# leggedrobotics/art_planner

Measured on AMD Instinct MI355X. Metric: validated states/sec on 400x400@0.04m map (sample + validity check), higher is better.
Workload: dtype f32; 1 GPU; C2: lazy_prm_star_min_update front end, 400x400@0.04m Perlin terrain (seed 1234) + 12 obstacles, YAML robot, batch sampler + validity checker; map=400x400@0.04, lanes=1

## Files before the change

### art_planner_amd/_capi.py

```python
from __future__ import annotations

import ctypes as C
import os

_HERE = os.path.dirname(os.path.abspath(__file__))
LIB_PATH = os.path.join(_HERE, "csrc", "libartp.so")
if os.environ.get("ARTP_LIB"):
    LIB_PATH = os.path.abspath(os.environ["ARTP_LIB"])

SYMBOLS = [
    "artp_params_defaults", "artp_params_yaml", "artp_status_string", "artp_last_error",
    "artp_device_arch", "artp_create", "artp_destroy", "artp_set_stream", "artp_use_own_stream",
    "artp_synchronize", "artp_set_lane", "artp_get_lane", "artp_map_version",
    "artp_upload_layer", "artp_update_layer_rect", "artp_update_layer_rects", "artp_check_boxes", "artp_check_boxes_dev",
    "artp_validate_states", "artp_validate_states_dev", "artp_set_persistent_latency", "artp_persistent_latency_stats", "artp_upload_sampler_layers",
    "artp_sample_states", "artp_sample_states_dev", "artp_sample_and_validate_dev",
    "artp_sample_and_validate", "artp_reachability_map", "artp_reachability_map_dev", "artp_reachability_poses",
    "artp_reachability_halo", "artp_field_params_defaults", "artp_field_compute", "artp_field_dist", "artp_field_dist_dev",
    "artp_field_path", "artp_field_edge_costs", "artp_field_stats", "artp_field_update", "artp_field_update_stats",
    "artp_field_destroy", "artp_field_learned_params_defaults", "artp_field_compute_learned", "artp_field_learned_stats",
    "artp_field_update_learned", "artp_field_learned_update_stats", "artp_field_block_moves", "artp_field_unblock",
    "artp_field_blocked_count", "artp_field_blocked", "artp_field_plan", "artp_field_plan_stats", "artp_field_plan_round_tile_runs",
    "artp_clearance_params_defaults", "artp_clearance_map", "artp_clearance_map_dev",
    "artp_field_clearance_params_defaults", "artp_field_compute_clearance", "artp_field_clearance",
    "artp_field_update_clearance", "artp_field_clearance_update_stats",
    "artp_check_motions_last_valid", "artp_check_motions_last_valid_dev",
    "artp_set_z_bounds", "artp_set_few_edges", "artp_set_edge_passes", "artp_cost_set_fc_path", "artp_check_motions", "artp_check_motions_dev", "artp_check_edges_interp",
    "artp_check_edges_interp_dev", "artp_compact_valid_dev", "artp_compact_valid_indices_dev", "artp_sample_states_at_dev",
    "artp_pack_edge_results_dev", "artp_cost_update_map_dev", "artp_pack_valid_bits_dev", "artp_indices_from_bits_dev",
    "artp_materialise_from_bits_dev",
    "artp_shard_first_index", "artp_group_create", "artp_group_unique_id", "artp_group_create_rank",
    "artp_group_destroy", "artp_group_last_error", "artp_group_world_size", "artp_group_local_count",
    "artp_group_rank", "artp_group_ctx", "artp_group_ranks_seen", "artp_group_configure",
    "artp_group_sample_and_validate_step", "artp_group_step_buffers", "artp_group_exchange_edges",
    "artp_group_edge_buffers", "artp_group_synchronize", "artp_group_abort",
    "artp_algorithmic_vertices_dev",
    "artp_debug_pipeline_counters", "artp_debug_partner_table", "artp_roadmap_params_defaults",
    "artp_roadmap_build", "artp_roadmap_stats", "artp_roadmap_export", "artp_roadmap_solve", "artp_roadmap_destroy",
    "artp_roadmap_revalidate", "artp_roadmap_set_query", "artp_roadmap_simplify_path", "artp_roadmap_grow",
    "artp_roadmap_solve_until", "artp_roadmap_set_density_map", "artp_roadmap_solve_many",
    "artp_preprocessed_reweight_dev",
    "artp_preprocess_params_defaults", "artp_preprocess_params_yaml", "artp_preprocess_map",
    "artp_preprocess_map_ex", "artp_preprocessed_change",
    "artp_preprocessed_get_layer", "artp_preprocessed_install", "artp_preprocessed_destroy",
    "artp_inpaint_layer", "artp_cost_set_hole_filling", "artp_cost_set_external_query",
    "artp_cost_blob_bytes", "artp_cost_load_weights", "artp_cost_update_map_layer",
    "artp_cost_update_map", "artp_cost_query", "artp_cost_query_dev", "artp_cost_get_features", "artp_cost_debug_query_cells",
    "artp_cost_debug_forms",
    "artp_cost_blob_bytes_version", "artp_cost_feature_channels", "artp_cost_get_features_c", "artp_cost_fc_path", "artp_set_r3_extent", "artp_telea_inpaint_u8",
    "artp_tree_params_defaults", "artp_tree_create", "artp_tree_grow", "artp_tree_solve", "artp_tree_stats",
# ... 192 lines not shown
    L.artp_field_destroy.restype = None
    L.artp_field_block_moves.argtypes = [vp, vp, vp, sz, C.POINTER(C.c_uint64)]
    L.artp_field_unblock.argtypes = [vp, vp, C.POINTER(C.c_uint64)]
    L.artp_field_blocked_count.argtypes = [vp, C.POINTER(C.c_uint64)]
    L.artp_field_blocked.argtypes = [vp, vp]
    L.artp_field_plan.argtypes = [vp, vp, sz, i32, vp, vp, vp, vp, vp, sz]
    L.artp_field_plan_stats.argtypes = [vp, C.POINTER(FieldPlanStats)]
    L.artp_field_plan_round_tile_runs.argtypes = [vp, vp, sz, C.POINTER(sz)]
    L.artp_clearance_params_defaults.argtypes = [C.POINTER(ClearanceParams)]
    L.artp_clearance_params_defaults.restype = None
    for name in ("artp_clearance_map", "artp_clearance_map_dev"):
        getattr(L, name).argtypes = [vp, C.POINTER(ClearanceParams), i32, i32, i32, vp, i32, vp]
    L.artp_field_clearance_params_defaults.argtypes = [C.POINTER(FieldClearanceParams)]
    L.artp_field_clearance_params_defaults.restype = None
    L.artp_field_compute_clearance.argtypes = [vp, C.POINTER(FieldClearanceParams), i32, vp, vp, i32, vp, sz, i32,
                                               C.POINTER(vp)]
    L.artp_field_clearance.argtypes = [vp, vp]
    L.artp_field_update_clearance.argtypes = [vp, vp, i32, vp, i32]
    L.artp_field_clearance_update_stats.argtypes = [vp, C.POINTER(FieldClearanceUpdateStats)]
    L.artp_map_version.argtypes = [vp]
    L.artp_map_version.restype = C.c_uint64
    L.artp_set_z_bounds.argtypes = [vp, dbl, dbl]
    L.artp_set_few_edges.argtypes = [vp, i32]
    L.artp_set_persistent_latency.argtypes = [vp, i32]
    L.artp_persistent_latency_stats.argtypes = [vp, C.POINTER(u64 * 2)]
    L.artp_set_edge_passes.argtypes = [vp, i32, i32]
    L.artp_cost_set_fc_path.argtypes = [vp, i32]
    for name in ("artp_check_motions_last_valid", "artp_check_motions_last_valid_dev"):
        getattr(L, name).argtypes = [vp, vp, vp, sz, vp, vp, vp]
    for name in ("artp_check_motions", "artp_check_motions_dev"):
        getattr(L, name).argtypes = [vp, vp, vp, sz, vp]
    for name in ("artp_check_edges_interp", "artp_check_edges_interp_dev"):
        getattr(L, name).argtypes = [vp, vp, vp, sz, vp, vp]
    L.artp_compact_valid_dev.argtypes = [vp, vp, vp, sz, vp, vp]
    L.artp_compact_valid_indices_dev.argtypes = [vp, vp, sz, vp, vp]
    L.artp_sample_states_at_dev.argtypes = [vp, u64, u64, vp, vp, sz, vp]
    L.artp_materialise_from_bits_dev.argtypes = [vp, u64, vp, i32, sz, sz, vp, sz, vp, vp]
    L.artp_pack_edge_results_dev.argtypes = [vp, vp, vp, vp, vp, sz, vp, vp]
    L.artp_pack_valid_bits_dev.argtypes = [vp, vp, sz, vp]
    L.artp_indices_from_bits_dev.argtypes = [vp, vp, sz, vp, vp]
    L.artp_shard_first_index.argtypes = [u64, i32, i32, u64]
    L.artp_shard_first_index.restype = u64
    L.artp_group_create.argtypes = [C.POINTER(i32), i32, C.POINTER(Params), i32, C.POINTER(vp)]
    L.artp_group_unique_id.argtypes = [vp]
    L.artp_group_create_rank.argtypes = [i32, i32, i32, vp, C.POINTER(Params), C.POINTER(vp)]
    L.artp_group_destroy.argtypes = [vp]
# ... 100 lines not shown
```

### art_planner_amd/context.py

```python
from __future__ import annotations

import ctypes as C
from typing import Optional

import numpy as np

from . import _capi


def make_params(kind="yaml", **overrides) -> _capi.Params:
    L = _capi.load()
    p = _capi.Params()
    (L.artp_params_yaml if kind == "yaml" else L.artp_params_defaults)(C.byref(p))
    for k, v in overrides.items():
        setattr(p, k, v)
    return p


def _f32F(a) -> np.ndarray:
    return np.asfortranarray(a, dtype=np.float32)


class Context:

# ... 86 lines not shown
        valid = np.empty(n, np.uint8)
        detail = np.empty((n, 6), np.int8) if want_detail else None
        self._chk(self.L.artp_validate_states(self.h, se3.ctypes.data, n, valid.ctypes.data,
                                              detail.ctypes.data if want_detail else None),
                  "artp_validate_states")
        return (valid, detail) if want_detail else valid

    def sample_states(self, seed, first_index, n):
        out = np.empty((n, 7), np.float64)
        self._chk(self.L.artp_sample_states(self.h, seed, first_index, n, out.ctypes.data),
                  "artp_sample_states")
        return out

    def set_persistent_latency(self, enabled=True):
        self._chk(self.L.artp_set_persistent_latency(self.h, 1 if enabled else 0), "artp_set_persistent_latency")

    def persistent_latency_stats(self):
        out = (C.c_uint64 * 2)()
        self._chk(self.L.artp_persistent_latency_stats(self.h, C.byref(out)), "artp_persistent_latency_stats")
        return {"launches": int(out[0]), "requests": int(out[1])}

    def set_few_edges(self, enabled=True):
        self._chk(self.L.artp_set_few_edges(self.h, 1 if enabled else 0), "artp_set_few_edges")

    def set_edge_passes(self, two_pass=True, coarse_stride=0):
        self._chk(self.L.artp_set_edge_passes(self.h, 1 if two_pass else 0, coarse_stride), "artp_set_edge_passes")

    def check_motions(self, s1, s2):
        s1 = np.ascontiguousarray(s1, np.float64).reshape(-1, 7)
        s2 = np.ascontiguousarray(s2, np.float64).reshape(-1, 7)
        valid = np.empty(s1.shape[0], np.uint8)
        self._chk(self.L.artp_check_motions(self.h, s1.ctypes.data, s2.ctypes.data, s1.shape[0],
                                            valid.ctypes.data), "artp_check_motions")
        return valid

    def set_z_bounds(self, z_low, z_high):
        self._chk(self.L.artp_set_z_bounds(self.h, float(z_low), float(z_high)), "artp_set_z_bounds")
        self.z_bounds = (float(z_low), float(z_high))

    def set_r3_extent(self, max_extent):
        self._chk(self.L.artp_set_r3_extent(self.h, float(max_extent)), "artp_set_r3_extent")

    def check_motions_last_valid(self, s1, s2):
        s1 = np.ascontiguousarray(s1, np.float64).reshape(-1, 7)
        s2 = np.ascontiguousarray(s2, np.float64).reshape(-1, 7)
        n = s1.shape[0]
# ... 169 lines not shown

    def check_boxes_dev(self, slot, box, poses_t, hit_t, ec_t=None):
        box = np.ascontiguousarray(box, np.float32)
        self._chk(self.L.artp_check_boxes_dev(self.h, slot, box.ctypes.data, poses_t.data_ptr(),
                                              poses_t.shape[0], hit_t.data_ptr(),
                                              ec_t.data_ptr() if ec_t is not None else None),
                  "artp_check_boxes_dev")

    def compact_valid_dev(self, se3_t, valid_t, out_t, count_t):
        self._chk(self.L.artp_compact_valid_dev(self.h, se3_t.data_ptr(), valid_t.data_ptr(), se3_t.shape[0],
                                                out_t.data_ptr(), count_t.data_ptr()), "artp_compact_valid_dev")

    def algorithmic_vertices_dev(self, se3_t) -> int:
        v = C.c_uint64(0)
        self._chk(self.L.artp_algorithmic_vertices_dev(self.h, se3_t.data_ptr(), se3_t.shape[0], C.byref(v)),
                  "artp_algorithmic_vertices_dev")
        return v.value

    def pipeline_counters(self):
        out = (C.c_uint64 * 8)()
        self._chk(self.L.artp_debug_pipeline_counters(self.h, C.byref(out)), "artp_debug_pipeline_counters")
        return {"torso_queued": out[0], "feet_queued": out[4], "exact_grouping": out[1], "feet_plane_stage": out[5],
                "feet_partner_pass": out[6],
                "torso_staged_pass": out[2]}

    def partner_table(self, slot, shape):
        r = C.c_int(0)
        self._chk(self.L.artp_debug_partner_table(self.h, slot, None, 0, C.byref(r)), "artp_debug_partner_table")
        if r.value == 0:
            return None, 0
        out = np.empty(shape[0] * shape[1], np.uint8)
        self._chk(self.L.artp_debug_partner_table(self.h, slot, out.ctypes.data, out.size, C.byref(r)),
                  "artp_debug_partner_table")
        return out.reshape(shape[1], shape[0]), r.value

    def preprocess_map(self, elevation, len_x, len_y, pos_x=0.0, pos_y=0.0, traversability=None, kind="yaml",
                       observed=None, vertices=None, **overrides):
        p = _capi.PreprocessParams()
        (self.L.artp_preprocess_params_yaml if kind == "yaml" else self.L.artp_preprocess_params_defaults)(C.byref(p))
        for k, v in overrides.items():
            setattr(p, k, v)
        e = _f32F(elevation)
        t = _f32F(traversability) if traversability is not None else None
        o = _f32F(observed) if observed is not None else None
        vs = np.ascontiguousarray(vertices, np.float64).reshape(-1, 7) if vertices is not None else None
        inp = _capi.PreprocessInputs(e.ctypes.data, t.ctypes.data if t is not None else None,
                                     o.ctypes.data if o is not None else None,
# ... 174 lines not shown
```

### art_planner_amd/csrc/artp_capi.hip

```cpp
#include "../../include/artp_c.h"

#include <hip/hip_runtime.h>
#include <hipcub/hipcub.hpp>

#include <cmath>
#include <cstdio>
#include <atomic>
#include <chrono>
#include <cstdlib>
#include <cstring>
#include <mutex>
#include <string>
#include <array>
#include <vector>

#include "device_scratch.h"
#include "pipeline.h"
#include "cost_kernels.h"

using namespace artp;

#define ARTP_FEW_STATES 16
#define ARTP_SVC_MAX_STATES 2
#define FEW_EDGE_S1 0
#define FEW_EDGE_S2 (ARTP_FEW_EDGES * 7 * sizeof(double))
#define FEW_EDGE_LAST_T (2 * ARTP_FEW_EDGES * 7 * sizeof(double))
#define FEW_EDGE_LAST_STATE (FEW_EDGE_LAST_T + ARTP_FEW_EDGES * sizeof(double))
#define FEW_EDGE_AUX (FEW_EDGE_LAST_STATE + ARTP_FEW_EDGES * 7 * sizeof(double))
#define FEW_EDGE_STATUS (FEW_EDGE_AUX + ARTP_FEW_EDGES * sizeof(uint32_t))
#define FEW_EDGE_BLOCK_BYTES (FEW_EDGE_STATUS + ARTP_FEW_EDGES)
#define ARTP_MAX_LANES 4

struct artp_ctx {
  int device = 0;
  hipStream_t own_stream = nullptr;
  hipStream_t stream = nullptr;
  artp_params params{};
  RobotDev robot{};
  MapGeom geom{};
  bool have_geom = false;
  std::atomic<uint64_t> map_version{0};
  FieldDev field[2]{};
  float* field_data[2] = {nullptr, nullptr};
  size_t field_elems[2] = {0, 0};
  bool have_field[2] = {false, false};
  void* rect_stage_host = nullptr;
  void* rect_stage_dev = nullptr;
  size_t rect_stage_cap = 0;
  hipEvent_t rect_stage_done = nullptr;
  hipEvent_t map_written = nullptr;
  hipEvent_t lane_mark[4] = {nullptr, nullptr, nullptr, nullptr};
  uint64_t map_write_seq = 0;
  uint64_t map_seen[4] = {0, 0, 0, 0};
  SamplerDev sampler{};
// ... 57 lines not shown
  char* pin_edges = nullptr;
  char* pin_edges_dev = nullptr;
  FewEdgeSync* d_few_sync = nullptr;
  int* d_error = nullptr;
  unsigned long long* d_count = nullptr;
  void* tmp[8] = {nullptr, nullptr, nullptr, nullptr, nullptr, nullptr, nullptr, nullptr};
  size_t tmp_cap[8] = {0, 0, 0, 0, 0, 0, 0, 0};
  void* cub_tmp = nullptr;
  size_t cub_cap = 0;
  int32_t* clear_offs[33] = {};
  uint32_t clear_n[33] = {};
  struct lane_state {
    bool init = false;
    hipStream_t own_stream = nullptr, stream = nullptr;
    unsigned long long* d_count = nullptr;
    int* d_error = nullptr;
    void* tmp[8] = {nullptr, nullptr, nullptr, nullptr, nullptr, nullptr, nullptr, nullptr};
    size_t tmp_cap[8] = {0, 0, 0, 0, 0, 0, 0, 0};
    void* cub_tmp = nullptr;
    size_t cub_cap = 0;
  };
  lane_state lanes[ARTP_MAX_LANES];
  int cur_lane = 0;
  bool have_weights = false;
  int cost_net = 0;
  half8* d_convw[5] = {nullptr, nullptr, nullptr, nullptr, nullptr};
  float* d_convb[5] = {nullptr, nullptr, nullptr, nullptr, nullptr};
  float* d_c12 = nullptr;
  unsigned char* d_c12m = nullptr;
  int conv12_mfma = 1;
  half8* d_convw_chunk[3] = {nullptr, nullptr, nullptr};
  half8* d_convw_p32 = nullptr;
  float* d_fc = nullptr;
  char* d_fc_mfma = nullptr;
  int feet_dense = 0;
  double r3_extent_override = 0.0;
  int fc_mfma = 1;
  int fc_selfcheck = -1;
  float fc_selfcheck_err = 0.f;
  half_t* d_act[2] = {nullptr, nullptr};
  size_t act_cap = 0;
  half_t* d_feat = nullptr;
  size_t feat_cap = 0;
  float* d_map_f32 = nullptr;
  size_t map_cap = 0;
  CostMapGeom cost_geom{};
// ... 182 lines not shown
  std::lock_guard<std::mutex> lock(mu);
  int* have = nullptr;
  for (auto& e : set)
    if (e.first.first == c->device && e.first.second == fn) have = &e.second;
  if (have && *have >= (int)bytes) return ARTP_OK;
  HIP_TRY(c, hipFuncSetAttribute(fn, hipFuncAttributeMaxDynamicSharedMemorySize, (int)bytes));
  if (have)
    *have = (int)bytes;
  else
    set.push_back({{c->device, fn}, (int)bytes});
  return ARTP_OK;
}

#define ARTP_OPT_IN(c, kernel, bytes)                                                       \
  do {                                                                                      \
    const int _rc = opt_in_lds((c), reinterpret_cast<const void*>(kernel), (bytes));        \
    if (_rc != ARTP_OK) return _rc;                                                         \
  } while (0)

int set_kernel_lds(artp_ctx* c) {
  ARTP_OPT_IN(c, check_boxes_kernel<1>, lds_full(c));
  ARTP_OPT_IN(c, validate_states_kernel<1>, lds_full(c));
  ARTP_OPT_IN(c, plane_stage_kernel<1>, lds_full(c));
  ARTP_OPT_IN(c, validate_few_kernel, lds_few(c));
  ARTP_OPT_IN(c, check_motions_few_kernel, lds_few(c));
  ARTP_OPT_IN(c, validate_service_kernel, lds_few(c));
  ARTP_OPT_IN(c, check_motions_pool_kernel, lds_few(c));
  ARTP_OPT_IN(c, (resolve_boxes_kernel<ARTP_WAVES_PER_BLOCK, 64, 3>), lds_scan(c));
  ARTP_OPT_IN(c, (resolve_boxes_kernel<ARTP_WAVES_PER_BLOCK, 16, 1>), lds_feet(c));
  ARTP_OPT_IN(c, (resolve_boxes_kernel<ARTP_WAVES_PER_BLOCK, 64, 2>), lds_feet_wave(c));
  return ARTP_OK;
}

int grid_full(const artp_ctx* c, size_t tasks) {
  size_t per_cu = (160 * 1024) / (lds_full(c) ? lds_full(c) : 1);
  if (per_cu > 16) per_cu = 16;
  if (per_cu < 1) per_cu = 1;
  size_t g = (size_t)c->n_cus * per_cu;
  if (tasks && tasks < g) g = tasks;
  return (int)(g ? g : 1);
}
int grid_scan(const artp_ctx* c, size_t lds) {
  size_t per_cu = (160 * 1024) / (lds ? lds : 1);
  if (per_cu > 8) per_cu = 8;
  if (per_cu < 1) per_cu = 1;
  return (int)((size_t)c->n_cus * per_cu);
// ... 157 lines not shown
  t.has_nan = f.has_nan;
  t.has_nonfinite = c->layer_has_nonfinite[slot];
  {
    unsigned off[ARTP_STRIDE_LEVELS + 1] = {0};
    for (int l = 0; l < ARTP_STRIDE_LEVELS; ++l) {
      const int s = 2 << l;
      off[l + 1] = off[l] + (unsigned)(((f.nW + s - 1) / s) * ((f.nD + s - 1) / s));
    }
    t.st = c->stride_buf[slot];
    t.st_off1 = off[1];
    t.st_off2 = off[2];
    hipLaunchKernelGGL(stride_tables_kernel, dim3((off[3] + 255) / 256), dim3(256), 0, c->stream, t.mm, t.fl, t.stride,
                       f.nW, f.nD, off[1], off[2], off[3], c->stride_buf[slot]);
    HIP_TRY(c, hipGetLastError());
  }
  const int rc_partner = pr ? partner_update_end(c, slot, *pr) : build_partner_table_full(c, slot);
  if (rc_partner != ARTP_OK) return rc_partner;
  t.valid = 1;
  return ARTP_OK;
}

int ensure_recs(artp_ctx* c, size_t n) { return ensure_tmp(c, 7, n * sizeof(PoseRec)); }

int launch_validate_pipeline(artp_ctx* c, const double* se3, size_t n, uint8_t* valid, bool recs_ready = false) {
  if (n >= (1ull << 32)) {
    c->last_error = "batch too large (state index is 32 bit)";
    return ARTP_ERR_INVALID_ARG;
  }
  int rc = ensure_recs(c, n);
  if (rc) return rc;
  PoseRec* recs = static_cast<PoseRec*>(c->tmp[7]);
  if (!recs_ready)
    hipLaunchKernelGGL(pose_rec_kernel, dim3((unsigned)((n + 255) / 256)), dim3(256), 0, c->stream, c->field[0], se3, n,
                       recs);
  const size_t per_block_states = 64 * ARTP_CLASSIFY_SUB;
  const size_t n_blocks = (n + per_block_states - 1) / per_block_states;
  const size_t seg_t = ((n_blocks + ARTP_NSUB - 1) / ARTP_NSUB) * per_block_states;
  rc = ensure_tmp(c, 4, 5 * ARTP_NSUB * seg_t * sizeof(PendingBox));
  if (rc) return rc;
  const size_t ctr_bytes = 128 + (size_t)2 * ARTP_NSUB * 128;
  rc = ensure_tmp(c, 5, ctr_bytes + ((5 + 4 + 4) * n + 5 * (size_t)ARTP_NSUB * seg_t) * sizeof(unsigned) + 64);
  if (rc) return rc;
  PipelineQueues q;
  q.q1 = static_cast<PendingBox*>(c->tmp[4]);
  q.counters = static_cast<unsigned long long*>(c->tmp[5]);
  q.sub = q.counters + 16;
  q.seg_t = seg_t;
  q.q2 = reinterpret_cast<unsigned*>(static_cast<char*>(c->tmp[5]) + ctr_bytes);
  q.q3 = q.q2 + 5 * n;
  q.q5 = q.q3 + 4 * n;
  q.q4 = q.q5 + 4 * n;
  q.q6 = q.q4 + 4 * (size_t)ARTP_NSUB * seg_t;
  q.feet_base = (unsigned long long)ARTP_NSUB * seg_t;
  HIP_TRY(c, hipMemsetAsync(q.counters, 0, ctr_bytes, c->stream));
  const size_t per_block = 64 * ARTP_CLASSIFY_SUB;
  hipLaunchKernelGGL(classify_states_kernel, dim3((unsigned)((n + per_block - 1) / per_block)),
                     dim3(ARTP_CLASSIFY_THREADS), 0, c->stream,
                     c->field[0], c->field[1], c->tables[0], c->tables[1], c->geom, c->robot, (const PoseRec*)recs, n,
                     valid, q);
#ifdef ARTP_VARIANTS
  if (c->feet_dense)
    hipLaunchKernelGGL(feet_stream2_kernel<ARTP_STREAM_WAVES>, dim3(grid_sub(c, ARTP_FEET_WAVES_PER_SIMD)), dim3(64 * ARTP_STREAM_WAVES), 0,
                       c->stream, c->field[1], c->robot, q, valid);
  else
#endif
    hipLaunchKernelGGL(feet_stream_kernel<ARTP_STREAM_WAVES>, dim3(grid_sub(c, ARTP_FEET_WAVES_PER_SIMD)), dim3(64 * ARTP_STREAM_WAVES), 0,
                       c->stream, c->field[1], c->robot, q, valid);
  hipLaunchKernelGGL(feet_lane_kernel, dim3((unsigned)c->n_cus * 8), dim3(ARTP_LANE_THREADS), 0, c->stream,
                     c->field[1], c->robot, q, valid);
  {
    const ScratchCaps caps_stream{0, 0, 0, 0};
    const size_t lds_stream = 0;
    hipLaunchKernelGGL((resolve_boxes_kernel<ARTP_WAVES_PER_BLOCK, 64, 0>), dim3(grid_sub(c, ARTP_TORSO_WGS_PER_CU)),
                       dim3(64 * ARTP_WAVES_PER_BLOCK), lds_stream, c->stream, c->field[0], c->robot, q, valid,
                       caps_stream, c->d_error, c->tables[0].valid ? c->tables[0].mm : (const float2*)nullptr);
  }
  hipLaunchKernelGGL((resolve_boxes_kernel<ARTP_WAVES_PER_BLOCK, 64, 3>), dim3(grid_scan(c, lds_scan(c))),
                     dim3(64 * ARTP_WAVES_PER_BLOCK), lds_scan(c), c->stream, c->field[0], c->robot, q, valid,
                     c->caps_scan, c->d_error);
  hipLaunchKernelGGL((resolve_boxes_kernel<ARTP_WAVES_PER_BLOCK, 16, 1>), dim3(grid_scan(c, lds_feet(c))),
                     dim3(64 * ARTP_WAVES_PER_BLOCK), lds_feet(c), c->stream, c->field[1], c->robot, q, valid,
                     c->caps_feet, c->d_error);
  hipLaunchKernelGGL((resolve_boxes_kernel<ARTP_WAVES_PER_BLOCK, 64, 2>), dim3(grid_scan(c, lds_feet_wave(c))),
                     dim3(64 * ARTP_WAVES_PER_BLOCK), lds_feet_wave(c), c->stream, c->field[1], c->robot, q, valid,
                     c->caps_feet_wave, c->d_error);
  hipLaunchKernelGGL(plane_stage_kernel<1>, dim3(grid_full(c, 0)), dim3(64), lds_full(c), c->stream,
                     c->field[0], c->field[1], c->robot, q, valid, c->caps_full, c->d_error);
  HIP_TRY(c, hipGetLastError());
  return ARTP_OK;
}

int check_error_flag(artp_ctx* c) {
  int flag = 0;
  HIP_TRY(c, hipMemcpyAsync(&flag, c->d_error, sizeof(int), hipMemcpyDeviceToHost, c->stream));
  HIP_TRY(c, hipStreamSynchronize(c->stream));
  if (flag) {
    HIP_TRY(c, hipMemsetAsync(c->d_error, 0, sizeof(int), c->stream));
    c->last_error = "a box window exceeded the LDS tile capacity";
    return ARTP_ERR_CAPACITY;
  }
  return ARTP_OK;
}

}

extern "C" {

void artp_params_defaults(artp_params* p) {
  p->torso_length = 1.05; p->torso_width = 0.55; p->torso_height = 0.2;
  p->torso_off_x = 0.0; p->torso_off_y = 0.0; p->torso_off_z = 0.0;
// ... 209 lines not shown
      void *pe = nullptr, *ped = nullptr;
      std::vector<FewEdgeSync> armed(ARTP_FEW_EDGES, FewEdgeSync{0xffffffffu, 0u, 0u, {0u}});
      void *pi = nullptr, *pid = nullptr;
      if (hipHostMalloc(&pi, 2 * ARTP_FEW_EDGES * 7 * sizeof(double), hipHostMallocMapped) == hipSuccess &&
          hipHostGetDevicePointer(&pid, pi, 0) == hipSuccess) {
        c->pin_edges_in = static_cast<char*>(pi);
        c->pin_edges_in_dev = static_cast<char*>(pid);
      } else if (pi) {
        (void)hipHostFree(pi);
      }
      if (!c->pin_edges_in ||
          hipHostMalloc(&pe, FEW_EDGE_BLOCK_BYTES, hipHostMallocMapped) != hipSuccess ||
          hipHostGetDevicePointer(&ped, pe, 0) != hipSuccess ||
          hipMalloc(reinterpret_cast<void**>(&c->d_few_sync), ARTP_FEW_EDGES * sizeof(FewEdgeSync)) != hipSuccess ||
          hipMemcpy(c->d_few_sync, armed.data(), ARTP_FEW_EDGES * sizeof(FewEdgeSync), hipMemcpyHostToDevice) != hipSuccess) {
        if (pe) (void)hipHostFree(pe);
        (void)hipHostFree(ps);
        (void)hipHostFree(pl);
        artp_destroy(c);
        return ARTP_ERR_HIP;
      }
      c->pin_edges = static_cast<char*>(pe);
      c->pin_edges_dev = static_cast<char*>(ped);
    }
    c->pin_states = static_cast<double*>(ps);
    c->pin_labels = static_cast<volatile uint8_t*>(pl);
    c->pin_states_dev = static_cast<double*>(psd);
    c->pin_labels_dev = static_cast<uint8_t*>(pld);
    const char* e = std::getenv("ARTP_NO_POLL");
    c->poll_labels = !(e && e[0] == '1');
#ifdef ARTP_VARIANTS
    if (const char* fd = std::getenv("ARTP_FEET_DENSE")) c->feet_dense = fd[0] != '0';
    if (const char* pw = std::getenv("ARTP_POOL_WGS")) {
      const long v = std::strtol(pw, nullptr, 10);
      if (v >= 1 && v <= ARTP_POOL_MAX_WGS) c->pool_wgs = (unsigned)v;
    }
#endif
  }
  fill_robot(c);
  *out = c;
  return ARTP_OK;
}

void artp_destroy(artp_ctx* c) {
  if (!c) return;
  (void)hipSetDevice(c->device);
// ... 38 lines not shown
  if (c->d_fc) (void)hipFree(c->d_fc);
  if (c->d_fc_mfma) (void)hipFree(c->d_fc_mfma);
  if (c->d_c12) (void)hipFree(c->d_c12);
  if (c->d_c12m) (void)hipFree(c->d_c12m);
  for (int l = 0; l < 3; ++l)
    if (c->d_convw_chunk[l]) (void)hipFree(c->d_convw_chunk[l]);
  if (c->d_convw_p32) (void)hipFree(c->d_convw_p32);
  for (int l = 0; l < 2; ++l)
    if (c->d_act[l]) (void)hipFree(c->d_act[l]);
  if (c->d_feat) (void)hipFree(c->d_feat);
  if (c->d_map_f32) (void)hipFree(c->d_map_f32);
  if (c->d_diff) (void)hipFree(c->d_diff);
  if (c->svc) (void)hipHostFree(c->svc);
  if (c->svc_stream) (void)hipStreamDestroy(c->svc_stream);
  if (c->svc_after_map) (void)hipEventDestroy(c->svc_after_map);
  if (c->pool_stream) (void)hipStreamDestroy(c->pool_stream);
  if (c->pool_after_map) (void)hipEventDestroy(c->pool_after_map);
  if (c->pool_mb) (void)hipFree(c->pool_mb);
  if (c->pool_resp) (void)hipHostFree(c->pool_resp);
  if (c->pool_ctl) (void)hipFree(c->pool_ctl);
  if (c->pin_edges) (void)hipHostFree(c->pin_edges);
  if (c->pin_edges_in) (void)hipHostFree(c->pin_edges_in);
  if (c->d_few_sync) (void)hipFree(c->d_few_sync);
  if (c->pin_states) (void)hipHostFree(c->pin_states);
  if (c->pin_labels) (void)hipHostFree(const_cast<uint8_t*>(c->pin_labels));
  delete c;
}

int artp_set_stream(artp_ctx* c, void* hip_stream) {
  if (!c) return ARTP_ERR_INVALID_ARG;
  std::lock_guard<std::recursive_mutex> lock(c->mu);
  c->stream = static_cast<hipStream_t>(hip_stream);
  if (c->map_written) {
    HIP_TRY(c, hipSetDevice(c->device));
    HIP_TRY(c, hipStreamWaitEvent(c->stream, c->map_written, 0));
  }
  return ARTP_OK;
}

int artp_use_own_stream(artp_ctx* c) {
  if (!c) return ARTP_ERR_INVALID_ARG;
  std::lock_guard<std::recursive_mutex> lock(c->mu);
  c->stream = c->own_stream;
  if (c->map_written) {
    HIP_TRY(c, hipSetDevice(c->device));
    HIP_TRY(c, hipStreamWaitEvent(c->stream, c->map_written, 0));
// ... 817 lines not shown
    c->last_error = "edge batch expands to 2^32 or more states: split it";
    return ARTP_ERR_CAPACITY;
  }
  const uint32_t total = (uint32_t)plan.total;
  const bool want_last = want_last_;
  if (want_last) HIP_TRY(c, hipMemsetAsync(first_bad, 0xff, n * sizeof(uint32_t), c->stream));
  size_t eb = ((size_t)total + 255) / 256;
  if (eb > (size_t)c->n_cus * 32) eb = (size_t)c->n_cus * 32;
  if (two_pass_possible && plan.total >= 24ull * n) {
    auto run_pass = [&](int pass, const uint32_t* offs, uint32_t tot) -> int {
      if (tot == 0) return ARTP_OK;
      size_t pb = ((size_t)tot + 255) / 256;
      if (pb > (size_t)c->n_cus * 32) pb = (size_t)c->n_cus * 32;
      int r = ensure_tmp(c, 3, (size_t)tot * (sizeof(uint32_t) + 1) + 64);
      if (r) return r;
      r = ensure_recs(c, tot);
      if (r) return r;
      uint32_t* edge_of = static_cast<uint32_t*>(c->tmp[3]);
      uint8_t* ex_valid = reinterpret_cast<uint8_t*>(edge_of + tot);
      hipLaunchKernelGGL(expand_edges_recs_kernel, dim3((unsigned)pb), dim3(256), 0, c->stream, c->field[0], mode, s1, s2, n,
                         offs, (const uint32_t*)aux, (const SlerpEdge*)d_slerp, static_cast<PoseRec*>(c->tmp[7]), edge_of,
                         pass, (uint32_t)c->edge_coarse_stride);
      HIP_TRY(c, hipGetLastError());
      r = launch_validate_pipeline(c, nullptr, tot, ex_valid, true);
      if (r) return r;
      hipLaunchKernelGGL(reduce_edges_kernel, dim3((unsigned)pb), dim3(256), 0, c->stream, (const uint8_t*)ex_valid,
                         (const uint32_t*)edge_of, offs, n, valid);
      HIP_TRY(c, hipGetLastError());
      return ARTP_OK;
    };
    rc = run_pass(1, offsets1, (uint32_t)plan.total1);
    if (rc) return rc;
    HIP_TRY(c, hipMemsetAsync(d_total1, 0, sizeof(unsigned long long), c->stream));
    hipLaunchKernelGGL(coarse_pass2_counts_kernel, dim3((unsigned)blocks), dim3(256), 0, c->stream, (const uint32_t*)aux,
                       (const uint8_t*)valid, n, (uint32_t)c->edge_coarse_stride, counts1, d_total1);
    HIP_TRY(c, hipGetLastError());
    cap = c->cub_cap;
    HIP_TRY(c, hipcub::DeviceScan::ExclusiveSum(c->cub_tmp, cap, counts1, offsets1, (int)(n + 1), c->stream));
    unsigned long long total2 = 0;
    HIP_TRY(c, hipMemcpyAsync(&total2, d_total1, sizeof(total2), hipMemcpyDeviceToHost, c->stream));
    HIP_TRY(c, hipStreamSynchronize(c->stream));
    return run_pass(2, offsets1, (uint32_t)total2);
  }
  if (total != 0) {
    rc = ensure_tmp(c, 3, (size_t)total * (sizeof(uint32_t) + 1) + 64);
    if (rc) return rc;
    rc = ensure_recs(c, total);
    if (rc) return rc;
    uint32_t* edge_of = static_cast<uint32_t*>(c->tmp[3]);
    uint8_t* ex_valid = reinterpret_cast<uint8_t*>(edge_of + total);
    hipLaunchKernelGGL(expand_edges_recs_kernel, dim3((unsigned)eb), dim3(256), 0, c->stream, c->field[0], mode, s1, s2, n,
                       (const uint32_t*)offsets, (const uint32_t*)aux, (const SlerpEdge*)d_slerp,
                       static_cast<PoseRec*>(c->tmp[7]), edge_of);
    HIP_TRY(c, hipGetLastError());
    rc = launch_validate_pipeline(c, nullptr, total, ex_valid, true);
    if (rc) return rc;
    hipLaunchKernelGGL(reduce_edges_kernel, dim3((unsigned)eb), dim3(256), 0, c->stream,
                       (const uint8_t*)ex_valid, (const uint32_t*)edge_of, (const uint32_t*)offsets, n, valid);
    if (want_last)
      hipLaunchKernelGGL(reduce_edges_first_bad_kernel, dim3((unsigned)eb), dim3(256), 0, c->stream,
                         (const uint8_t*)ex_valid, (const uint32_t*)edge_of, (const uint32_t*)offsets,
                         (const uint32_t*)aux, n, first_bad);
    HIP_TRY(c, hipGetLastError());
  }
  if (want_last) {
    hipLaunchKernelGGL(last_valid_kernel, dim3((unsigned)blocks), dim3(256), 0, c->stream, s1, s2, n,
                       (const uint32_t*)aux, (const uint32_t*)first_bad, last_t, last_state);
    HIP_TRY(c, hipGetLastError());
  }
  return ARTP_OK;
}

static double few_edges_task_estimate(const artp_ctx* c, int mode, const double* s1, const double* s2, size_t n,
                                      double* max_per_edge) {
  double total = 0.0, mx = 1.0;
  const double ex = 2.0 * c->geom.len_x, ey = 2.0 * c->geom.len_y, ez = c->z_high - c->z_low;
  const double seg = (c->r3_extent_override > 0.0 ? c->r3_extent_override : std::sqrt(ex * ex + ey * ey + ez * ez)) * 0.01;
  for (size_t e = 0; e < n; ++e) {
// ... 300 lines not shown
                     last_t ? d_last_t : nullptr, last_state ? d_last_state : nullptr);
  if (rc) return rc;
  HIP_TRY(c, hipMemcpyAsync(valid, d_valid, n, hipMemcpyDeviceToHost, c->stream));
  if (aux_out) HIP_TRY(c, hipMemcpyAsync(aux_out, d_aux, n * sizeof(uint32_t), hipMemcpyDeviceToHost, c->stream));
  if (last_t) HIP_TRY(c, hipMemcpyAsync(last_t, d_last_t, n * sizeof(double), hipMemcpyDeviceToHost, c->stream));
  if (last_t && last_state)
    HIP_TRY(c, hipMemcpyAsync(last_state, d_last_state, n * 7 * sizeof(double), hipMemcpyDeviceToHost, c->stream));
  return check_error_flag(c);
}

int artp_set_edge_passes(artp_ctx* c, int two_pass, int coarse_stride) {
  if (!c || (coarse_stride != 0 && coarse_stride < 2)) return ARTP_ERR_INVALID_ARG;
  std::lock_guard<std::recursive_mutex> lock(c->mu);
  c->edge_two_pass = two_pass != 0;
  c->edge_coarse_stride = coarse_stride ? coarse_stride : ARTP_COARSE_STRIDE;
  return ARTP_OK;
}
int artp_set_few_edges(artp_ctx* c, int enabled) {
  if (!c) return ARTP_ERR_INVALID_ARG;
  std::lock_guard<std::recursive_mutex> lock(c->mu);
  c->few_edges = enabled != 0;
  return ARTP_OK;
}
int artp_check_motions_dev(artp_ctx* c, const double* s1, const double* s2, size_t n, uint8_t* valid) {
  return run_edges_dev(c, 0, s1, s2, n, valid, nullptr);
}
int artp_check_motions(artp_ctx* c, const double* s1, const double* s2, size_t n, uint8_t* valid) {
  return run_edges_host(c, 0, s1, s2, n, valid, nullptr);
}
int artp_check_motions_last_valid_dev(artp_ctx* c, const double* s1, const double* s2, size_t n, uint8_t* valid,
                                      double* last_valid_t, double* last_valid_se3) {
  if (n && !last_valid_t) return ARTP_ERR_INVALID_ARG;
  return run_edges_dev(c, 0, s1, s2, n, valid, nullptr, last_valid_t, last_valid_se3);
}
int artp_check_motions_last_valid(artp_ctx* c, const double* s1, const double* s2, size_t n, uint8_t* valid,
                                  double* last_valid_t, double* last_valid_se3) {
  if (n && !last_valid_t) return ARTP_ERR_INVALID_ARG;
  return run_edges_host(c, 0, s1, s2, n, valid, nullptr, last_valid_t, last_valid_se3);
}
int artp_check_edges_interp_dev(artp_ctx* c, const double* s1, const double* s2, size_t n,
                                uint8_t* valid, uint32_t* n_interp_out) {
  return run_edges_dev(c, 1, s1, s2, n, valid, n_interp_out);
}
int artp_check_edges_interp(artp_ctx* c, const double* s1, const double* s2, size_t n, uint8_t* valid,
                            uint32_t* n_interp_out) {
  return run_edges_host(c, 1, s1, s2, n, valid, n_interp_out);
}


namespace {
struct Se3Row { double v[7]; };
}

int artp_debug_pipeline_counters(artp_ctx* c, uint64_t out[8]) {
  if (!c || !out) return ARTP_ERR_INVALID_ARG;
  std::lock_guard<std::recursive_mutex> lock(c->mu);
  if (!c->tmp[5]) return ARTP_ERR_NO_MAP;
  HIP_TRY(c, hipSetDevice(c->device));
  uint64_t raw[16 + 2 * ARTP_NSUB * 16];
  HIP_TRY(c, hipMemcpyAsync(raw, c->tmp[5], sizeof(raw), hipMemcpyDeviceToHost, c->stream));
  HIP_TRY(c, hipStreamSynchronize(c->stream));
  for (int k = 0; k < 8; ++k) out[k] = raw[k];
  out[0] = out[4] = out[2] = out[7] = 0;
  for (int s = 0; s < ARTP_NSUB; ++s) {
    out[0] += raw[16 + (size_t)s * 16];
    out[4] += raw[16 + (size_t)(ARTP_NSUB + s) * 16];
    out[2] += raw[16 + (size_t)s * 16 + 2];
    out[7] += raw[16 + (size_t)(ARTP_NSUB + s) * 16 + 2];
  }
  return ARTP_OK;
}

int artp_debug_partner_table(artp_ctx* c, int slot, uint8_t* out, size_t out_bytes, int* radius) {
  if (!c || slot < 0 || slot > 1 || !radius) return ARTP_ERR_INVALID_ARG;
  std::lock_guard<std::recursive_mutex> lock(c->mu);
  if (!c->have_field[slot]) return ARTP_ERR_NO_MAP;
  const FieldDev& f = c->field[slot];
  *radius = f.partner_flags ? f.partner_R : 0;
  if (!out || !f.partner_flags) return ARTP_OK;
  const size_t need = (size_t)f.nW * f.nD;
  if (out_bytes < need) return ARTP_ERR_INVALID_ARG;
  HIP_TRY(c, hipSetDevice(c->device));
  HIP_TRY(c, hipMemcpyAsync(out, f.partner_flags, need, hipMemcpyDeviceToHost, c->stream));
  HIP_TRY(c, hipStreamSynchronize(c->stream));
  return ARTP_OK;
// ... 1226 lines not shown
```

### art_planner_amd/csrc/pipeline.h

```cpp
#pragma once

#include <hip/hip_fp16.h>

#include "kernels.h"

namespace artp {

#define ARTP_TABLE_LEVELS 4

struct TablesDev {
  const float2* mm;
  const unsigned char* fl;
  unsigned stride;
  int has_nan;
  int has_nonfinite;
  int valid;
  const unsigned* st;
  unsigned st_off1, st_off2;
};

#define ARTP_STRIDE_LEVELS 3

__global__ void __launch_bounds__(256)
table_level0_kernel(const float* __restrict__ data, int n, float2* __restrict__ mm, unsigned char* __restrict__ fl) {
// ... 1124 lines not shown
        } else if (gl == 0) {
          const unsigned long long slot = atomicAdd(&q.counters[1], 1ull);
          q.q2[slot] = (unsigned)item;
        }
      }
    }
    if (decided && gl == 0) {
      const bool ok = (rec.kind & 1u) ? (result != 0) : (result == 0);
      if (!ok) valid[rec.state] = 0;
    }
    wave_lds_sync();
  }
#ifdef ARTP_STAGE_TIMING
  if (gl == 0) {
    for (int k = 0; k < 8; ++k) atomicAdd(&g_stage_cycles[G == 64 ? 0 : 1][k], t_acc[k]);
    if (PASS == 0)
      for (int k = 0; k < 8; ++k) atomicAdd(&g_torso_counts[k], t_cnt[k]);
    atomicAdd(&g_stage_cycles[G == 64 ? 0 : 1][8], (unsigned long long)(clock64() - t_begin));
    atomicAdd(&g_stage_cycles[G == 64 ? 0 : 1][9], 1ull);
  }
#endif
}

template <int WAVES>
__global__ void __launch_bounds__(64 * WAVES)
plane_stage_kernel(FieldDev fb, FieldDev ff, RobotDev rb, PipelineQueues q, uint8_t* __restrict__ valid,
                   ScratchCaps caps, int* __restrict__ error_flag) {
  extern __shared__ __attribute__((aligned(16))) char smem[];
  const int lane = threadIdx.x & 63;
  const WaveScratch s = carve_scratch(smem, threadIdx.x >> 6, caps);
  const unsigned long long count = q.counters[1];
  const unsigned long long stride = (unsigned long long)gridDim.x * WAVES;
  for (unsigned long long item = (unsigned long long)blockIdx.x * WAVES + (threadIdx.x >> 6); item < count;
       item += stride) {
    const PendingBox rec = q.q1[q.q2[item]];
    if (valid[rec.state] == 0) continue;
    BoxHF b;
    box_from_record(rec, rb, b);
    const bool foot = (rec.kind & 1u) != 0;
    WindowStats w;
    if (foot)
      wave_scan_window(ff, b, s, lane, w);
    else
      wave_scan_window(fb, b, s, lane, w);
    const int T = wave_compact_triangles<true>(b, s, lane);
    int result;
    if (T < 0)
      result = (foot ? wave_plane_stage_unlisted(ff, b, s, lane) : wave_plane_stage_unlisted(fb, b, s, lane)) ? 1 : 0;
    else
      result = (T > 0 && (foot ? wave_plane_stage(ff, b, s, lane, T) : wave_plane_stage(fb, b, s, lane, T))) ? 1 : 0;
    if (lane == 0) {
      const bool ok = (rec.kind & 1u) ? (result != 0) : (result == 0);
      if (!ok) valid[rec.state] = 0;
    }
    wave_lds_sync();
  }
}

#ifdef ARTP_VARIANTS
#include "pipeline_variants.h"
#endif

}
```

### include/artp_c.h

```cpp
#ifndef ARTP_C_H
#define ARTP_C_H

#include <stddef.h>
#include <stdint.h>

#ifdef __cplusplus
extern "C" {
#endif

typedef struct artp_ctx artp_ctx;

typedef enum {
  ARTP_OK = 0,
  ARTP_ERR_INVALID_ARG = -1,
  ARTP_ERR_NO_DEVICE = -2,
  ARTP_ERR_HIP = -3,
  ARTP_ERR_NO_MAP = -4,
  ARTP_ERR_CAPACITY = -5,
  ARTP_ERR_NO_WEIGHTS = -6,
  ARTP_ERR_TIMEOUT = -7,
  ARTP_ERR_COMM = -8,
  ARTP_ERR_COST_FUNC = -9
} artp_status;

// ... 179 lines not shown
                                 const uint32_t* mask, int mask_on_device, const int* sources, size_t n_sources, int reverse,
                                 artp_field** out);
int artp_field_clearance(artp_field* f, uint16_t* d2_out);
typedef struct artp_field_clearance_update_stats_t {
  uint64_t changed_words, removed_nodes, added_nodes, dead_nodes, hop_dead_nodes, unsupport_rounds, dist_rounds,
      hop_rounds, tile_launches, reached_nodes;
  uint64_t clearance_tiles;
  uint64_t changed_d2;
  uint64_t repriced_slots;
  uint64_t changed_slots;
  uint64_t weight_tiles;
  double clearance_ms, reprice_ms;
  double passes_ms;
} artp_field_clearance_update_stats_t;
int artp_field_update_clearance(artp_field* f, const uint32_t* new_mask, int mask_on_device, const int sub_rect[4],
                                int refresh_heights);
int artp_field_clearance_update_stats(artp_field* f, artp_field_clearance_update_stats_t* out);

int artp_set_z_bounds(artp_ctx* ctx, double z_low, double z_high);
int artp_set_r3_extent(artp_ctx* ctx, double max_extent);
int artp_check_motions(artp_ctx* ctx, const double* s1, const double* s2, size_t n, uint8_t* valid);
int artp_set_few_edges(artp_ctx* ctx, int enabled);
int artp_set_edge_passes(artp_ctx* ctx, int two_pass, int coarse_stride);
int artp_check_motions_dev(artp_ctx* ctx, const double* s1, const double* s2, size_t n,
                           uint8_t* valid);
int artp_check_motions_last_valid(artp_ctx* ctx, const double* s1, const double* s2, size_t n, uint8_t* valid,
                                  double* last_valid_t, double* last_valid_se3);
int artp_check_motions_last_valid_dev(artp_ctx* ctx, const double* s1, const double* s2, size_t n, uint8_t* valid,
                                      double* last_valid_t, double* last_valid_se3);
int artp_check_edges_interp(artp_ctx* ctx, const double* s1, const double* s2, size_t n,
                            uint8_t* valid, uint32_t* n_interp_out);
int artp_check_edges_interp_dev(artp_ctx* ctx, const double* s1, const double* s2, size_t n,
                                uint8_t* valid, uint32_t* n_interp_out);

int artp_compact_valid_dev(artp_ctx* ctx, const double* se3, const uint8_t* valid, size_t n,
                           double* out_se3, uint64_t* n_out_dev);
int artp_compact_valid_indices_dev(artp_ctx* ctx, const uint8_t* valid, size_t n, uint32_t* out_idx,
                                   uint64_t* n_out_dev);
int artp_sample_states_at_dev(artp_ctx* ctx, uint64_t seed, uint64_t base_index, const uint32_t* idx,
                              const uint64_t* count_dev, size_t cap, double* se3_out);
int artp_pack_valid_bits_dev(artp_ctx* ctx, const uint8_t* valid, size_t n, uint64_t* bits_out);
int artp_materialise_from_bits_dev(artp_ctx* ctx, uint64_t seed, const uint64_t* bits, int n_ranks,
                                   size_t words_per_rank, size_t prefix_bits, const uint64_t* base_index, size_t cap,
                                   double* se3_out, uint64_t* counts_dev);
int artp_indices_from_bits_dev(artp_ctx* ctx, const uint64_t* bits, size_t n, uint32_t* out_idx, uint64_t* n_out_dev);
int artp_pack_edge_results_dev(artp_ctx* ctx, const uint8_t* valid, const uint32_t* edge_i, const uint32_t* edge_j,
// ... 174 lines not shown
```

Baseline: 4.324 billion states/s.

## Collapse tail validation stages into one rare-boxes kernel when hinted queue is small

Adds an adaptive tail path. The last stage writes a hint word to mapped host memory holding the count of leftover boxes. If a previous call on the same map version reported a small tail, the next call skips the feet lane kernel and the scan, feet-wave and plane-stage kernels, and runs one rare_boxes_kernel that resolves all queued boxes wave by wave. This cuts kernel launches and per-stage overhead for sparse tails, but relies on a stale hint from a prior batch, so a large tail can end up on a slower single-wave-per-box path.

```diff
diff --git a/art_planner_amd/_capi.py b/art_planner_amd/_capi.py
--- a/art_planner_amd/_capi.py
+++ b/art_planner_amd/_capi.py
@@ -25,7 +25,7 @@
     "artp_field_clearance_params_defaults", "artp_field_compute_clearance", "artp_field_clearance",
     "artp_field_update_clearance", "artp_field_clearance_update_stats",
     "artp_check_motions_last_valid", "artp_check_motions_last_valid_dev",
-    "artp_set_z_bounds", "artp_set_few_edges", "artp_set_edge_passes", "artp_cost_set_fc_path", "artp_check_motions", "artp_check_motions_dev", "artp_check_edges_interp",
+    "artp_set_z_bounds", "artp_set_few_edges", "artp_set_tail_mode", "artp_last_tail", "artp_set_edge_passes", "artp_cost_set_fc_path", "artp_check_motions", "artp_check_motions_dev", "artp_check_edges_interp",
     "artp_check_edges_interp_dev", "artp_compact_valid_dev", "artp_compact_valid_indices_dev", "artp_sample_states_at_dev",
     "artp_pack_edge_results_dev", "artp_cost_update_map_dev", "artp_pack_valid_bits_dev", "artp_indices_from_bits_dev",
     "artp_materialise_from_bits_dev",
@@ -264,6 +264,8 @@
     L.artp_map_version.restype = C.c_uint64
     L.artp_set_z_bounds.argtypes = [vp, dbl, dbl]
     L.artp_set_few_edges.argtypes = [vp, i32]
+    L.artp_set_tail_mode.argtypes = [vp, i32]
+    L.artp_last_tail.argtypes = [vp]
     L.artp_set_persistent_latency.argtypes = [vp, i32]
     L.artp_persistent_latency_stats.argtypes = [vp, C.POINTER(u64 * 2)]
     L.artp_set_edge_passes.argtypes = [vp, i32, i32]
diff --git a/art_planner_amd/context.py b/art_planner_amd/context.py
--- a/art_planner_amd/context.py
+++ b/art_planner_amd/context.py
@@ -132,6 +132,12 @@
 
     def set_few_edges(self, enabled=True):
         self._chk(self.L.artp_set_few_edges(self.h, 1 if enabled else 0), "artp_set_few_edges")
+
+    def set_tail_mode(self, mode=0):
+        self._chk(self.L.artp_set_tail_mode(self.h, int(mode)), "artp_set_tail_mode")
+
+    def last_tail(self):
+        return int(self.L.artp_last_tail(self.h))
 
     def set_edge_passes(self, two_pass=True, coarse_stride=0):
         self._chk(self.L.artp_set_edge_passes(self.h, 1 if two_pass else 0, coarse_stride), "artp_set_edge_passes")
@@ -347,7 +353,7 @@
         self._chk(self.L.artp_debug_pipeline_counters(self.h, C.byref(out)), "artp_debug_pipeline_counters")
         return {"torso_queued": out[0], "feet_queued": out[4], "exact_grouping": out[1], "feet_plane_stage": out[5],
                 "feet_partner_pass": out[6],
-                "torso_staged_pass": out[2]}
+                "torso_staged_pass": out[2], "feet_lane_scan": out[7]}
 
     def partner_table(self, slot, shape):
         r = C.c_int(0)
diff --git a/art_planner_amd/csrc/artp_capi.hip b/art_planner_amd/csrc/artp_capi.hip
--- a/art_planner_amd/csrc/artp_capi.hip
+++ b/art_planner_amd/csrc/artp_capi.hip
@@ -30,6 +30,10 @@
 #define FEW_EDGE_STATUS (FEW_EDGE_AUX + ARTP_FEW_EDGES * sizeof(uint32_t))
 #define FEW_EDGE_BLOCK_BYTES (FEW_EDGE_STATUS + ARTP_FEW_EDGES)
 #define ARTP_MAX_LANES 4
+#define ARTP_TAIL_STATES 0
+#define ARTP_TAIL_EDGES_1 1
+#define ARTP_TAIL_EDGES_2 2
+#define ARTP_TAIL_KINDS 3
 
 struct artp_ctx {
   int device = 0;
@@ -133,6 +137,12 @@
   };
   lane_state lanes[ARTP_MAX_LANES];
   int cur_lane = 0;
+  int tail_mode = 0;
+  volatile unsigned* tail_hint = nullptr;
+  unsigned* tail_hint_dev = nullptr;
+  uint64_t tail_map_version[ARTP_MAX_LANES][ARTP_TAIL_KINDS] = {};
+  uint32_t tail_tag[ARTP_MAX_LANES][ARTP_TAIL_KINDS] = {};
+  int tail_last[ARTP_MAX_LANES] = {0, 0, 0, 0};
   bool have_weights = false;
   int cost_net = 0;
   half8* d_convw[5] = {nullptr, nullptr, nullptr, nullptr, nullptr};
@@ -361,6 +371,7 @@
   ARTP_OPT_IN(c, check_boxes_kernel<1>, lds_full(c));
   ARTP_OPT_IN(c, validate_states_kernel<1>, lds_full(c));
   ARTP_OPT_IN(c, plane_stage_kernel<1>, lds_full(c));
+  ARTP_OPT_IN(c, rare_boxes_kernel, lds_full(c));
   ARTP_OPT_IN(c, validate_few_kernel, lds_few(c));
   ARTP_OPT_IN(c, check_motions_few_kernel, lds_few(c));
   ARTP_OPT_IN(c, validate_service_kernel, lds_few(c));
@@ -564,7 +575,8 @@
 
 int ensure_recs(artp_ctx* c, size_t n) { return ensure_tmp(c, 7, n * sizeof(PoseRec)); }
 
-int launch_validate_pipeline(artp_ctx* c, const double* se3, size_t n, uint8_t* valid, bool recs_ready = false) {
+int launch_validate_pipeline(artp_ctx* c, const double* se3, size_t n, uint8_t* valid, bool recs_ready = false,
+                             int tail_kind = ARTP_TAIL_STATES) {
   if (n >= (1ull << 32)) {
     c->last_error = "batch too large (state index is 32 bit)";
     return ARTP_ERR_INVALID_ARG;
@@ -608,14 +620,38 @@
 #endif
     hipLaunchKernelGGL(feet_stream_kernel<ARTP_STREAM_WAVES>, dim3(grid_sub(c, ARTP_FEET_WAVES_PER_SIMD)), dim3(64 * ARTP_STREAM_WAVES), 0,
                        c->stream, c->field[1], c->robot, q, valid);
-  hipLaunchKernelGGL(feet_lane_kernel, dim3((unsigned)c->n_cus * 8), dim3(ARTP_LANE_THREADS), 0, c->stream,
-                     c->field[1], c->robot, q, valid);
+  const int lane_id = c->cur_lane;
+  const uint64_t map_v = c->map_version.load(std::memory_order_acquire) + 1;
+  const bool fresh = c->tail_map_version[lane_id][tail_kind] != map_v;
+  if (fresh) {
+    c->tail_map_version[lane_id][tail_kind] = map_v;
+    ++c->tail_tag[lane_id][tail_kind];
+  }
+  const unsigned hint_tag = c->tail_tag[lane_id][tail_kind] & 0xffu;
+  const size_t hint_at = 16 * (size_t)(lane_id * ARTP_TAIL_KINDS + tail_kind);
+  unsigned* hint_dev = c->tail_hint_dev + hint_at;
+  const unsigned rare_waves = (unsigned)grid_full(c, 0);
+  bool rare = c->tail_mode == 2;
+  if (c->tail_mode == 0 && !fresh) {
+    const unsigned word = c->tail_hint[hint_at];
+    rare = (word & 0xffu) == hint_tag && (word >> 8) <= rare_waves;
+  }
+  c->tail_last[lane_id] = rare ? 2 : 1;
+  if (!rare)
+    hipLaunchKernelGGL(feet_lane_kernel, dim3((unsigned)c->n_cus * 8), dim3(ARTP_LANE_THREADS), 0, c->stream,
+                       c->field[1], c->robot, q, valid);
   {
     const ScratchCaps caps_stream{0, 0, 0, 0};
     const size_t lds_stream = 0;
     hipLaunchKernelGGL((resolve_boxes_kernel<ARTP_WAVES_PER_BLOCK, 64, 0>), dim3(grid_sub(c, ARTP_TORSO_WGS_PER_CU)),
                        dim3(64 * ARTP_WAVES_PER_BLOCK), lds_stream, c->stream, c->field[0], c->robot, q, valid,
                        caps_stream, c->d_error, c->tables[0].valid ? c->tables[0].mm : (const float2*)nullptr);
+  }
+  if (rare) {
+    hipLaunchKernelGGL(rare_boxes_kernel, dim3(rare_waves), dim3(64), lds_full(c), c->stream, c->field[0], c->field[1],
+                       c->robot, q, valid, c->caps_full, c->d_error, hint_dev, hint_tag);
+    HIP_TRY(c, hipGetLastError());
+    return ARTP_OK;
   }
   hipLaunchKernelGGL((resolve_boxes_kernel<ARTP_WAVES_PER_BLOCK, 64, 3>), dim3(grid_scan(c, lds_scan(c))),
                      dim3(64 * ARTP_WAVES_PER_BLOCK), lds_scan(c), c->stream, c->field[0], c->robot, q, valid,
@@ -627,7 +663,7 @@
                      dim3(64 * ARTP_WAVES_PER_BLOCK), lds_feet_wave(c), c->stream, c->field[1], c->robot, q, valid,
                      c->caps_feet_wave, c->d_error);
   hipLaunchKernelGGL(plane_stage_kernel<1>, dim3(grid_full(c, 0)), dim3(64), lds_full(c), c->stream,
-                     c->field[0], c->field[1], c->robot, q, valid, c->caps_full, c->d_error);
+                     c->field[0], c->field[1], c->robot, q, valid, c->caps_full, c->d_error, hint_dev, hint_tag);
   HIP_TRY(c, hipGetLastError());
   return ARTP_OK;
 }
@@ -883,6 +919,20 @@
       }
       c->pin_edges = static_cast<char*>(pe);
       c->pin_edges_dev = static_cast<char*>(ped);
+    }
+    {
+      void *ph = nullptr, *phd = nullptr;
+      if (hipHostMalloc(&ph, ARTP_MAX_LANES * ARTP_TAIL_KINDS * 16 * sizeof(unsigned), hipHostMallocMapped) != hipSuccess ||
+          hipHostGetDevicePointer(&phd, ph, 0) != hipSuccess) {
+        if (ph) (void)hipHostFree(ph);
+        (void)hipHostFree(ps);
+        (void)hipHostFree(pl);
+        artp_destroy(c);
+        return ARTP_ERR_HIP;
+      }
+      std::memset(ph, 0xff, ARTP_MAX_LANES * ARTP_TAIL_KINDS * 16 * sizeof(unsigned));
+      c->tail_hint = static_cast<volatile unsigned*>(ph);
+      c->tail_hint_dev = static_cast<unsigned*>(phd);
     }
     c->pin_states = static_cast<double*>(ps);
     c->pin_labels = static_cast<volatile uint8_t*>(pl);
@@ -967,6 +1017,7 @@
   if (c->pin_edges) (void)hipHostFree(c->pin_edges);
   if (c->pin_edges_in) (void)hipHostFree(c->pin_edges_in);
   if (c->d_few_sync) (void)hipFree(c->d_few_sync);
+  if (c->tail_hint) (void)hipHostFree(const_cast<unsigned*>(c->tail_hint));
   if (c->pin_states) (void)hipHostFree(c->pin_states);
   if (c->pin_labels) (void)hipHostFree(const_cast<uint8_t*>(c->pin_labels));
   delete c;
@@ -1830,7 +1881,7 @@
                          offs, (const uint32_t*)aux, (const SlerpEdge*)d_slerp, static_cast<PoseRec*>(c->tmp[7]), edge_of,
                          pass, (uint32_t)c->edge_coarse_stride);
       HIP_TRY(c, hipGetLastError());
-      r = launch_validate_pipeline(c, nullptr, tot, ex_valid, true);
+      r = launch_validate_pipeline(c, nullptr, tot, ex_valid, true, pass == 2 ? ARTP_TAIL_EDGES_2 : ARTP_TAIL_EDGES_1);
       if (r) return r;
       hipLaunchKernelGGL(reduce_edges_kernel, dim3((unsigned)pb), dim3(256), 0, c->stream, (const uint8_t*)ex_valid,
                          (const uint32_t*)edge_of, offs, n, valid);
@@ -1861,7 +1912,7 @@
                        (const uint32_t*)offsets, (const uint32_t*)aux, (const SlerpEdge*)d_slerp,
                        static_cast<PoseRec*>(c->tmp[7]), edge_of);
     HIP_TRY(c, hipGetLastError());
-    rc = launch_validate_pipeline(c, nullptr, total, ex_valid, true);
+    rc = launch_validate_pipeline(c, nullptr, total, ex_valid, true, ARTP_TAIL_EDGES_1);
     if (rc) return rc;
     hipLaunchKernelGGL(reduce_edges_kernel, dim3((unsigned)eb), dim3(256), 0, c->stream,
                        (const uint8_t*)ex_valid, (const uint32_t*)edge_of, (const uint32_t*)offsets, n, valid);
@@ -2208,6 +2259,17 @@
   c->few_edges = enabled != 0;
   return ARTP_OK;
 }
+int artp_set_tail_mode(artp_ctx* c, int mode) {
+  if (!c || mode < 0 || mode > 2) return ARTP_ERR_INVALID_ARG;
+  std::lock_guard<std::recursive_mutex> lock(c->mu);
+  c->tail_mode = mode;
+  return ARTP_OK;
+}
+int artp_last_tail(artp_ctx* c) {
+  if (!c) return -1;
+  std::lock_guard<std::recursive_mutex> lock(c->mu);
+  return c->tail_last[c->cur_lane];
+}
 int artp_check_motions_dev(artp_ctx* c, const double* s1, const double* s2, size_t n, uint8_t* valid) {
   return run_edges_dev(c, 0, s1, s2, n, valid, nullptr);
 }
@@ -2247,6 +2309,7 @@
   HIP_TRY(c, hipMemcpyAsync(raw, c->tmp[5], sizeof(raw), hipMemcpyDeviceToHost, c->stream));
   HIP_TRY(c, hipStreamSynchronize(c->stream));
   for (int k = 0; k < 8; ++k) out[k] = raw[k];
+  out[1] += raw[3];
   out[0] = out[4] = out[2] = out[7] = 0;
   for (int s = 0; s < ARTP_NSUB; ++s) {
     out[0] += raw[16 + (size_t)s * 16];
diff --git a/art_planner_amd/csrc/pipeline.h b/art_planner_amd/csrc/pipeline.h
--- a/art_planner_amd/csrc/pipeline.h
+++ b/art_planner_amd/csrc/pipeline.h
@@ -1170,13 +1170,20 @@
 #endif
 }
 
+__device__ __forceinline__ void store_tail_hint(const PipelineQueues& q, unsigned* hint, unsigned tag) {
+  const unsigned long long n = fwd_total(q, 1) + fwd_total(q, 0) + q.counters[6] + q.counters[1];
+  *hint = (tag & 0xffu) | ((n > 0xffffffull ? 0xffffffu : (unsigned)n) << 8);
+}
+
 template <int WAVES>
 __global__ void __launch_bounds__(64 * WAVES)
 plane_stage_kernel(FieldDev fb, FieldDev ff, RobotDev rb, PipelineQueues q, uint8_t* __restrict__ valid,
-                   ScratchCaps caps, int* __restrict__ error_flag) {
+                   ScratchCaps caps, int* __restrict__ error_flag, unsigned* __restrict__ hint = nullptr,
+                   unsigned hint_tag = 0u) {
   extern __shared__ __attribute__((aligned(16))) char smem[];
   const int lane = threadIdx.x & 63;
   const WaveScratch s = carve_scratch(smem, threadIdx.x >> 6, caps);
+  if (hint != nullptr && blockIdx.x == 0 && threadIdx.x == 0) store_tail_hint(q, hint, hint_tag);
   const unsigned long long count = q.counters[1];
   const unsigned long long stride = (unsigned long long)gridDim.x * WAVES;
   for (unsigned long long item = (unsigned long long)blockIdx.x * WAVES + (threadIdx.x >> 6); item < count;
@@ -1205,6 +1212,59 @@
   }
 }
 
+template <bool EXITS_AND_F>
+__device__ __forceinline__ int rare_resolve_box(const FieldDev& f, const BoxHF& b, const WaveScratch& s, int lane,
+                                                bool exits_negative, unsigned long long* grouped) {
+  WindowStats w;
+  wave_scan_window(f, b, s, lane, w);
+  if (EXITS_AND_F) {
+    int result = 0, ec;
+    if (!exits_negative && decide_exits(b, w, result, ec)) return result;
+    if (wave_vertex_pass(f, b, s, lane, w.allFinite)) return 1;
+  }
+  if (lane == 0) atomicAdd(grouped, 1ull);
+  const int T = wave_compact_triangles<true>(b, s, lane);
+  if (T < 0) return wave_plane_stage_unlisted(f, b, s, lane) ? 1 : 0;
+  return (T > 0 && wave_plane_stage(f, b, s, lane, T)) ? 1 : 0;
+}
+
+__global__ void __launch_bounds__(64)
+rare_boxes_kernel(FieldDev fb, FieldDev ff, RobotDev rb, PipelineQueues q, uint8_t* __restrict__ valid,
+                  ScratchCaps caps, int* __restrict__ error_flag, unsigned* __restrict__ hint, unsigned hint_tag) {
+  extern __shared__ __attribute__((aligned(16))) char smem[];
+  const int lane = threadIdx.x;
+  const WaveScratch s = carve_scratch(smem, 0, caps);
+  if (hint != nullptr && blockIdx.x == 0 && lane == 0) store_tail_hint(q, hint, hint_tag);
+  const unsigned long long n4 = fwd_total(q, 1), n6 = fwd_total(q, 0), n5 = q.counters[6];
+  const unsigned long long count = n4 + n6 + n5;
+  for (unsigned long long it = blockIdx.x; it < count; it += gridDim.x) {
+    const int from = it < n4 ? 0 : (it < n4 + n6 ? 1 : 2);
+    const unsigned item = from == 0 ? fwd_item(q, 1, q.q4, it) : (from == 1 ? fwd_item(q, 0, q.q6, it - n4) : q.q5[it - n4 - n6]);
+    const PendingBox rec = q.q1[item];
+    if (valid[rec.state] == 0) continue;
+    BoxHF b;
+    box_from_record(rec, rb, b);
+    const int total = (b.maxX - b.minX + 1) * (b.maxZ - b.minZ + 1);
+    if (total > s.cap_verts) {
+      if (lane == 0) atomicExch(error_flag, 1);
+      continue;
+    }
+    const bool foot = (rec.kind & 1u) != 0;
+    int result;
+    if (from == 2)
+      result = rare_resolve_box<false>(ff, b, s, lane, true, &q.counters[3]);
+    else if (foot)
+      result = rare_resolve_box<true>(ff, b, s, lane, (rec.kind & ARTP_REC_EXITS_NEGATIVE) != 0, &q.counters[3]);
+    else
+      result = rare_resolve_box<true>(fb, b, s, lane, false, &q.counters[3]);
+    if (lane == 0) {
+      const bool ok = foot ? (result != 0) : (result == 0);
+      if (!ok) valid[rec.state] = 0;
+    }
+    wave_lds_sync();
+  }
+}
+
 #ifdef ARTP_VARIANTS
 #include "pipeline_variants.h"
 #endif
diff --git a/include/artp_c.h b/include/artp_c.h
--- a/include/artp_c.h
+++ b/include/artp_c.h
@@ -225,6 +225,8 @@
 int artp_check_motions(artp_ctx* ctx, const double* s1, const double* s2, size_t n, uint8_t* valid);
 int artp_set_few_edges(artp_ctx* ctx, int enabled);
 int artp_set_edge_passes(artp_ctx* ctx, int two_pass, int coarse_stride);
+int artp_set_tail_mode(artp_ctx* ctx, int mode);
+int artp_last_tail(artp_ctx* ctx);
 int artp_check_motions_dev(artp_ctx* ctx, const double* s1, const double* s2, size_t n,
                            uint8_t* valid);
 int artp_check_motions_last_valid(artp_ctx* ctx, const double* s1, const double* s2, size_t n, uint8_t* valid,
```

After: 4.426 billion states/s (median of 6 runs). 1.02x the previous value.
